# jglaser/metadynamics-plugin

Hardware: AMD Instinct MI355X
Metric: particle_cv_evals_per_s (higher is better)
Workload: dtype f32; 1 GPU; 1xMI355X: 10^6 particles, 2 lamellar CVs (8 Fourier modes each), 256^2 bias grid, well-tempered; particles_per_gpu=1000000, particles_global=1000000, n_cv=2, modes_per_cv=8, grid=256x256, stride=1, fast_trig=1, fast_trig_library_default=1, driver=host, mode=single

## Files before the change

### include/mtd_abi.h

```cpp
#ifndef MTD_ABI_H
#define MTD_ABI_H

#include <stddef.h>

#ifdef __cplusplus
extern "C" {
#endif

#define MTD_ABI_VERSION 1

typedef void *mtd_stream_t;

enum mtd_dtype { MTD_F32 = 0, MTD_F64 = 1 };

enum mtd_status
    {
    MTD_SUCCESS = 0,
    MTD_ERR_INVALID_ARGUMENT = -1,
    MTD_ERR_UNSUPPORTED = -2,
    MTD_ERR_NO_DEVICE = -3,
    MTD_ERR_COMM_TIMEOUT = -4,
    MTD_ERR_COLLECTIVE = -5
    };

// ... 70 lines not shown
                     const double *cv_max, const unsigned int *num_points, double W, double T_shift,
                     double T, unsigned int stride, int mode, int add_bias);
int mtd_metad_destroy(mtd_metad *m);

int mtd_metad_set_stride(mtd_metad *m, unsigned int stride);
int mtd_metad_set_add_hills(mtd_metad *m, int add_bias);
int mtd_metad_set_mode(mtd_metad *m, int mode);
int mtd_metad_set_sigma_inv(mtd_metad *m, const double *sigma_inv );
int mtd_metad_reset_histogram(mtd_metad *m, mtd_stream_t stream);

int mtd_metad_set_cv_source(mtd_metad *m, unsigned int cv, const double *d_partials, unsigned int n_partials,
                            unsigned int stride, unsigned int offset, double scale, double shift);

int mtd_metad_set_cv_value(mtd_metad *m, unsigned int cv, double value);

const double *mtd_metad_bias_device(const mtd_metad *m);
const double *mtd_metad_cv_device(const mtd_metad *m);

int mtd_metad_update_bias(mtd_metad *m, unsigned int timestep, mtd_stream_t stream);

int mtd_metad_update_phase_a(mtd_metad *m, unsigned int timestep, int *deposited, mtd_stream_t stream);
int mtd_metad_update_phase_b(mtd_metad *m, int deposited, mtd_stream_t stream);
int mtd_metad_delta_buffers(mtd_metad *m, double **d_real, unsigned int **d_count, unsigned int *num_elements);

int mtd_metad_get_state(mtd_metad *m, double *cv, double *bias, double *bias_potential, double *weight,
                        unsigned int *num_gaussians, unsigned int *num_out_of_bounds, mtd_stream_t stream);
double mtd_metad_sigma_determinant(const mtd_metad *m);
unsigned int mtd_metad_num_elements(const mtd_metad *m);

int mtd_metad_get_array(mtd_metad *m, int which, void *host_out, mtd_stream_t stream);
int mtd_metad_set_array(mtd_metad *m, int which, const void *host_in, mtd_stream_t stream);
int mtd_metad_set_num_gaussians(mtd_metad *m, unsigned int n, mtd_stream_t stream);
void *mtd_metad_device_array(mtd_metad *m, int which);
int mtd_metad_grid_touched(mtd_metad *m, mtd_stream_t stream);


int mtd_fused_cv_pass(mtd_metad *m, const mtd_lamellar_set *set, unsigned int n_particles, const void *d_postype,
                      int dtype, const mtd_box *global_box, double *d_partials, unsigned int *n_partials,
                      mtd_stream_t stream);

int mtd_fused_force_pass(mtd_metad *m, const mtd_lamellar_set *set, unsigned int n_particles, const void *d_postype,
                         void *const *d_force, int dtype, unsigned int n_global, const mtd_box *global_box,
                         unsigned int timestep, mtd_stream_t stream);

int mtd_fused_force_pass_slots(mtd_metad *m, const mtd_lamellar_set *set, const unsigned int *slots, unsigned int n_particles,
                               const void *d_postype, void *const *d_force, int dtype, unsigned int n_global,
                               const mtd_box *global_box, unsigned int timestep, mtd_stream_t stream);

int mtd_fused_step(mtd_metad *m, const mtd_lamellar_set *set, unsigned int n_particles, const void *d_postype,
                   void *const *d_force, int dtype, unsigned int n_global, const mtd_box *global_box, double *d_scratch,
                   unsigned int timestep, mtd_stream_t stream);
unsigned int mtd_fused_step_launches(const mtd_metad *m);
int mtd_fused_step_set_mode(mtd_metad *m, int mode);

int mtd_profile_force_begin(unsigned int n_launches);
int mtd_profile_force_end(double *durations_us, unsigned int capacity, unsigned int *n_out);

#define MTD_RCCL_ID_BYTES 128
#define MTD_ELEM_F64 1
#define MTD_ELEM_U32 2
typedef struct mtd_rccl mtd_rccl;
int mtd_rccl_unique_id(void *out_id);
int mtd_rccl_create(mtd_rccl **out, const void *unique_id, unsigned int rank, unsigned int world);
int mtd_comm_allreduce_large(mtd_rccl *r, void *d_buffer, size_t count, int elem, mtd_stream_t stream);
unsigned int mtd_rccl_world(const mtd_rccl *r);
unsigned int mtd_rccl_rank(const mtd_rccl *r);
int mtd_rccl_destroy(mtd_rccl *r);
const char *mtd_rccl_last_error(void);
int mtd_metad_update_bias_walkers(mtd_metad *m, mtd_rccl *walkers, unsigned int timestep, mtd_stream_t stream);


#define MTD_COMM_MAX_RANKS 8
#define MTD_COMM_HANDLE_BYTES 64

typedef struct mtd_comm mtd_comm;

int mtd_comm_create(mtd_comm **out, unsigned int rank, unsigned int world, unsigned int max_doubles);
int mtd_comm_handle(mtd_comm *c, void *out_handle);
int mtd_comm_connect(mtd_comm *c, const void *handles);
int mtd_comm_allreduce_small(mtd_comm *c, double *d_values, unsigned int n, mtd_stream_t stream);
int mtd_comm_status(mtd_comm *c, unsigned int *timeouts, mtd_stream_t stream);
#define MTD_COMM_MAX_SHARED 8
int mtd_comm_share(mtd_comm *c, size_t bytes, void **d_local, unsigned int *slot, void *out_handle);
int mtd_comm_open(mtd_comm *c, unsigned int slot, const void *handles, void **peers);
size_t mtd_comm_pull_bytes(size_t max_doubles);
int mtd_comm_pull_attach(mtd_comm *c, size_t max_doubles, void *const *in_peers, void *const *out_peers);
int mtd_comm_allreduce_pull(mtd_comm *c, double *d_buffer, size_t count, mtd_stream_t stream);
unsigned int mtd_comm_world(const mtd_comm *c);
unsigned int mtd_comm_rank(const mtd_comm *c);
int mtd_comm_destroy(mtd_comm *c);

int mtd_metad_set_comm(mtd_metad *m, mtd_comm *comm);


typedef struct mtd_mesh mtd_mesh;

int mtd_mesh_create(mtd_mesh **out, unsigned int nx, unsigned int ny, unsigned int nz, const double *mode,
                    unsigned int n_types, unsigned int max_particles);
int mtd_mesh_destroy(mtd_mesh *m);
int mtd_mesh_set_bug_compat(mtd_mesh *m, int on);
int mtd_mesh_set_keep_fourier(mtd_mesh *m, int on);
int mtd_mesh_set_cv_event(mtd_mesh *m, void *hip_event);
unsigned int mtd_mesh_num_cells(const mtd_mesh *m);

int mtd_mesh_compute_cv(mtd_mesh *m, unsigned int n_particles, const void *d_postype, int dtype, const mtd_box *box,
                        unsigned int n_global, const double **d_partials, unsigned int *n_partials, mtd_stream_t stream);
// ... 131 lines not shown
```

### metadynamics-plugin_amd/csrc/fused.hip

```cpp
#include <hip/hip_runtime.h>
#include <hip/hip_ext.h>

#ifdef MTD_STAMPS
__device__ unsigned long long g_stamps[64];
#define MTD_STAMP(slot, cond)                                                   \
    do                                                                          \
        {                                                                       \
        if (cond) g_stamps[slot] = wall_clock64();                              \
        } while (0)
extern "C" int mtd_debug_read_stamps(unsigned long long *host)
    {
    return (int)hipMemcpyFromSymbol(host, HIP_SYMBOL(g_stamps), sizeof(unsigned long long) * 64);
    }
#else
#define MTD_STAMP(slot, cond) do { } while (0)
#endif

#include "lamellar_host.hpp"
#include "metad_host.hpp"
#include "comm_host.hpp"

#include <cstdlib>
#include <cstring>
#include <map>
// ... 29 lines not shown
        apply_cells(c, b0, min(c.len, b0 + FCV_THREADS), blockIdx.x == 0, s_red);
        MTD_STAMP(1, blockIdx.x == 0 && threadIdx.x == 0);
        return;
        }
    const unsigned int block_id = blockIdx.x - n_apply_blocks;
    const unsigned int n_blocks = gridDim.x - n_apply_blocks;

    RawGroup<S4, U> first;
    const S4 *src = N ? postype : (const S4 *)partials;
    lam_load_group_nc<S4, U>(src, N ? N : 1u, block_id * FCV_THREADS + threadIdx.x, n_blocks * FCV_THREADS, first);
    const CvTableRegs tab = stage_cv_tables_request(a);
    stage_cv_tables_store(tab, s_coeff, s_mt);
    __syncthreads();
    MTD_STAMP(4, block_id == 0 && threadIdx.x == 0);
    float acc[NCV];
#pragma unroll
    for (int i = 0; i < NCV; ++i) acc[i] = 0.0f;
    lam_cv_accumulate<S4, NCV, FAST, U, ORTHO>(a, postype, N, block_id * FCV_THREADS + threadIdx.x, n_blocks * FCV_THREADS,
                                               s_coeff, s_mt, first, acc);
    MTD_STAMP(5, block_id == 0 && threadIdx.x == 0);
    lam_cv_block_reduce<NCV>(acc, s_wave, partials, block_id);
    MTD_STAMP(6, block_id == 0 && threadIdx.x == 0);
    if (COMM)
        {
        constexpr int NS = NCV < 3 ? NCV : 3;
        if (threadIdx.x < NS)
            ll_store(ck.ll + ((size_t)block_id * NS + threadIdx.x) * 2, ck.seq, partials[block_id * NCV + threadIdx.x]);
        if (block_id != 0 || threadIdx.x >= MTD_WAVE) return;
        double v[3] = { 0.0, 0.0, 0.0 };
        const bool expired = ll_collect_wave<NS>(ck, n_blocks, v);
        MTD_STAMP(7, threadIdx.x == 0);
        double tot[3] = { 0.0, 0.0, 0.0 };
#pragma unroll
        for (int i = 0; i < NS; ++i)
            {
            const double t = wave_sum(v[i]);
            tot[i] = expired ? comm_poison() : t;
            }
        MTD_STAMP(8, threadIdx.x == 0);
        comm_send_wave(ck, tot, NS);
        MTD_STAMP(9, threadIdx.x == 0);
        }
    }

constexpr int FF_STREAM_WAVES = FF_THREADS / MTD_WAVE - 1;
constexpr int FF_STREAM_THREADS = FF_STREAM_WAVES * MTD_WAVE;
constexpr int FF_U = 4;
template<typename S4, int NCV, bool FAST> struct ff_groups { static constexpr int value = 1; };
template<> struct ff_groups<float4, 1, true> { static constexpr int value = 2; };
template<> struct ff_groups<float4, 2, true> { static constexpr int value = 2; };
template<> struct ff_groups<float4, 1, false> { static constexpr int value = 2; };
template<> struct ff_groups<double4, 1, true> { static constexpr int value = 2; };
template<> struct ff_groups<double4, 1, false> { static constexpr int value = 2; };

template<typename S4, int NCV, bool FAST, int GROUPS, bool COMM, bool ORTHO>
__global__ __launch_bounds__(FF_THREADS, 4) void k_fused_force(const LamKArgs a, const S4 *__restrict__ postype, const ForcePtrs out,
                                                            const unsigned int N, const double two_over_n, const MetadCfg c,
                                                            const int deposit, const unsigned int n_grid_blocks, const CommK ck)
    {
    __shared__ ChainResult s_chain;
    __shared__ float s_wcoef[MTD_MAX_CV * MTD_MAX_TYPES];
    __shared__ double s_red[16];
    __shared__ ModeTables s_mt;

    const int wave = threadIdx.x >> 6;
    const int lane = threadIdx.x & 63;
    const bool grid_block = blockIdx.x < n_grid_blocks;
    const unsigned int block_id = blockIdx.x - n_grid_blocks;
    const unsigned int n_blocks = gridDim.x - n_grid_blocks;
    const unsigned int stride = n_blocks * FF_STREAM_THREADS;
    const unsigned int first = block_id * FF_STREAM_THREADS + (wave - 1) * MTD_WAVE + lane;
    const unsigned int first1 = first + FF_U * stride;

    ForceRegs<NCV, FF_U> R, R1;
    MTD_STAMP(16, blockIdx.x == 0 && threadIdx.x == 0);
    MTD_STAMP(24, blockIdx.x == n_grid_blocks && threadIdx.x == 0);
    constexpr int NCH = CHAIN_MAX_CV;
    ChainPre<NCH> pre;
    constexpr bool early = !COMM;
    float4 th = make_float4(0.f, 0.f, 0.f, 0.f), tq = th;
    float tc = 0.0f;
    if (wave == 0)
        {
        if (!grid_block)
            {
            if (lane < (int)a.n_modes)
                {
                th = a.h[lane];
                tq = a.q[lane];
                }
            if (lane < NCV * MTD_MAX_TYPES) tc = a.coeff[lane / MTD_MAX_TYPES][lane % MTD_MAX_TYPES];
            }
        if (early)
            chain_preload<NCH>(c, pre);
        else
            chain_preload<NCH, false>(c, pre);
        }
    RawGroup<S4, FF_U> raw0;
    if (wave != 0 && !grid_block && N) lam_force_request<S4, FF_U>(postype, N, first, stride, raw0);
    if (!grid_block)
        {
        if (wave == 0)
            {
            if (lane < (int)a.n_modes)
                {
                s_mt.h[lane] = th;
                s_mt.q[lane] = tq;
                }
            if (lane < NCV * MTD_MAX_TYPES) s_wcoef[lane] = tc;
            }
        lds_barrier();
        }
    MTD_STAMP(25, blockIdx.x == n_grid_blocks && threadIdx.x == 0);
    if (wave == 0)
        {
        ChainResult r;
        if constexpr (early)
            {
            double vi[3];
#pragma unroll
            for (int i = 0; i < NCH; ++i) vi[i] = (pre.x[i][0] + pre.x[i][1]) + (pre.x[i][2] + pre.x[i][3]);
            r = chain_wave(c, deposit != 0, true, nullptr, nullptr, false, &pre.patch, pre.patch_ok != 0, true, vi[0], vi[1], vi[2]);
            }
        else
            r = chain_wave(c, deposit != 0, true, &ck, nullptr, false, &pre.patch, pre.patch_ok != 0);
        MTD_STAMP(17, blockIdx.x == 0 && threadIdx.x == 0);
        MTD_STAMP(26, blockIdx.x == n_grid_blocks && threadIdx.x == 0);
        if (lane == 0) chain_share(s_chain, r);
        if (!grid_block && lane < NCV * MTD_MAX_TYPES)
            {
            const unsigned int cv = lane / MTD_MAX_TYPES;
            const unsigned int gs = cv < a.n_cv ? a.slot[cv] : 0u;
            const double b = gs == 0 ? r.bias[0] : (gs == 1 ? r.bias[1] : r.bias[2]);
            s_wcoef[lane] = (cv < a.n_cv) ? (float)((double)s_wcoef[lane] * b * two_over_n) : 0.0f;
            }
        }
    else if (!grid_block && N)
        {
        RawGroup<S4, FF_U> raw1;
        if (GROUPS > 1) lam_force_request<S4, FF_U>(postype, N, first1, stride, raw1);
        lam_force_unscaled_from<S4, NCV, FAST, FF_U, ORTHO>(a, N, first, stride, s_mt, raw0, R);
        if (GROUPS > 1) lam_force_unscaled_from<S4, NCV, FAST, FF_U, ORTHO>(a, N, first1, stride, s_mt, raw1, R1);
        MTD_STAMP(27, blockIdx.x == n_grid_blocks && threadIdx.x == 64);
        }
    lds_barrier();
    MTD_STAMP(18, blockIdx.x == 0 && threadIdx.x == 0);
    MTD_STAMP(28, blockIdx.x == n_grid_blocks && threadIdx.x == 64);

    if (grid_block)
        {
        const double2 sums = grid_first_pass_cells_256(c, s_chain, blockIdx.x);
        MTD_STAMP(19, blockIdx.x == 0 && threadIdx.x == 0);
        grid_first_pass_sums_256(c, blockIdx.x, sums, s_red);
        MTD_STAMP(20, blockIdx.x == 0 && threadIdx.x == 0);
        }
    else if (wave != 0 && N)
        {
        lam_force_store<S4, NCV, FF_U>(a, out, first, stride, s_wcoef, R);
        if (GROUPS > 1) lam_force_store<S4, NCV, FF_U>(a, out, first1, stride, s_wcoef, R1);
        MTD_STAMP(29, blockIdx.x == n_grid_blocks && threadIdx.x == 64);
        }

    if (blockIdx.x == 0 && wave == 0) publish_step(c, s_chain, deposit, nullptr, COMM ? &ck : nullptr);
    }

template<typename S4, bool FAST>
__global__ __launch_bounds__(FF_THREADS) void k_fused_force_general(const LamKArgs a, const S4 *__restrict__ postype, const ForcePtrs out,
                                                            const unsigned int N, const double two_over_n, const MetadCfg c,
                                                            const int deposit, const unsigned int n_grid_blocks)
    {
    __shared__ EvalShared sh;
    __shared__ float s_wcoef[MTD_MAX_CV * MTD_MAX_TYPES];
    __shared__ double s_red[16];
    __shared__ ModeTables s_mt;

    load_modes(a, s_mt, true);
    reduce_cv_sources(c, sh.cv, s_red);
    __syncthreads();
    evaluate_bias(c, sh, deposit != 0, true);

    if (blockIdx.x < n_grid_blocks)
        {
        const unsigned int g = blockIdx.x * FF_THREADS + threadIdx.x;
        double s1 = 0.0, s2 = 0.0;
        if (g < c.len)
            {
            const double dV = (c.W * sh.scal) * exp(-gauss_exponent(c, g, sh.cv));
            c.grid_delta[g] = dV;
            unsigned int hd = c.hist_delta[g];
            if (sh.on_grid && g == sh.bin)
                {
                hd += 1;
                c.hist_delta[g] = hd;
                c.sigma_grid_delta[g] += c.det_sigma;
                c.hist_gauss_delta[g] += 1;
                }
            const double R = c.rew[g] + (double)hd;
            c.rew[g] = R;
            s1 = R * dV;
            s2 = R;
            }
        s1 = block_sum(s1, s_red);
        s2 = block_sum(s2, s_red);
        if (threadIdx.x == 0)
            {
            c.gpart[2 * blockIdx.x] = s1;
            c.gpart[2 * blockIdx.x + 1] = s2;
            }
        }

    if (blockIdx.x == 0)
        {
        if (threadIdx.x < c.n_cv)
// ... 130 lines not shown
        MTD_LAUNCH_CHECK();
        return MTD_SUCCESS;
        });
    if (rc) return rc;
    m->pending_apply = 0;
    return MTD_SUCCESS;
    }

int mtd_fused_force_pass(mtd_metad *m, const mtd_lamellar_set *set, unsigned int n_particles, const void *d_postype,
                         void *const *d_force, int dtype, unsigned int n_global, const mtd_box *global_box,
                         unsigned int timestep, mtd_stream_t stream)
    {
    if (!m || !set) return MTD_ERR_INVALID_ARGUMENT;
    if (set->n_cv != m->cfg.n_cv) return MTD_ERR_UNSUPPORTED;
    return mtd_fused_force_pass_slots(m, set, nullptr, n_particles, d_postype, d_force, dtype, n_global, global_box, timestep, stream);
    }

int mtd_fused_force_pass_slots(mtd_metad *m, const mtd_lamellar_set *set, const unsigned int *slots, unsigned int n_particles,
                               const void *d_postype, void *const *d_force, int dtype, unsigned int n_global,
                               const mtd_box *global_box, unsigned int timestep, mtd_stream_t stream)
    {
    if (!m) return MTD_ERR_INVALID_ARGUMENT;
    LamKArgs k;
    int rc = fill_kargs(k, set, global_box);
    if (rc) return rc;
    if (!d_force || n_global == 0 || (n_particles && !d_postype)) return MTD_ERR_INVALID_ARGUMENT;
    if (dtype != MTD_F32 && dtype != MTD_F64) return MTD_ERR_INVALID_ARGUMENT;
    if (set->n_cv > m->cfg.n_cv) return MTD_ERR_UNSUPPORTED;
    if (!slots && set->n_cv != m->cfg.n_cv) return MTD_ERR_INVALID_ARGUMENT;
    if (slots)
        {
        if (m->comm) return MTD_ERR_UNSUPPORTED;
        for (unsigned int c = 0; c < set->n_cv; ++c)
            {
            if (slots[c] >= m->cfg.n_cv) return MTD_ERR_INVALID_ARGUMENT;
            k.slot[c] = (unsigned char)slots[c];
            }
        }
    hipStream_t s = (hipStream_t)stream;
    rc = metad_flush(m, s);
    if (rc) return rc;
    ForcePtrs out;
    for (unsigned int c = 0; c < MTD_MAX_CV; ++c) out.f[c] = nullptr;
    for (unsigned int c = 0; c < set->n_cv; ++c)
        {
        if (!d_force[c] && n_particles) return MTD_ERR_INVALID_ARGUMENT;
        out.f[c] = d_force[c];
        }
    const int dep = deposit_due(m, timestep);
    const unsigned int n_grid = dep ? m->cfg.n_gblocks : 0;
    const double two_over_n = 2.0 / (double)n_global;
    const bool fast = lam_fast_trig(k) != 0;
    static const bool force_general = std::getenv("MTD_FUSED_GENERAL") != nullptr;
    CommK ck;
    std::memset(&ck, 0, sizeof(ck));
    if (m->comm)
        {
        if (m->cfg.n_cv > (unsigned int)CHAIN_MAX_CV || force_general) return MTD_ERR_UNSUPPORTED;
        rc = comm_current(m->comm, ck);
        if (rc) return rc;
        }
    if (m->cfg.n_cv <= (unsigned int)CHAIN_MAX_CV && !force_general)
        {
        hipEvent_t ev_start = nullptr, ev_stop = nullptr;
        const bool timed = force_profile_next(ev_start, ev_stop);
        dispatch_s4_fast(dtype, fast, [&](auto s4, auto fast_c)
            {
            using S4 = typename decltype(s4)::type;
            constexpr bool FAST = decltype(fast_c)::value;
            dispatch_count<CHAIN_MAX_CV>(set->n_cv, [&](auto n)
                {
                constexpr int NCV = decltype(n)::value, G = ff_groups<S4, NCV, FAST>::value;
                const unsigned int per_block = FF_STREAM_THREADS * FF_U * G;
                unsigned int fblocks = (n_particles + per_block - 1) / per_block;
                if (fblocks == 0 && n_grid == 0) fblocks = 1;
                const unsigned int grid = n_grid + fblocks;
                dispatch_bool(m->comm != nullptr, [&](auto comm_c)
                    {
                    dispatch_bool(k.ortho != 0, [&](auto ortho_c)
                        {
                        const auto kernel = k_fused_force<S4, NCV, FAST, G, decltype(comm_c)::value, decltype(ortho_c)::value>;
                        if (timed)
                            hipExtLaunchKernelGGL(kernel, dim3(grid), dim3(FF_THREADS), 0, s, ev_start, ev_stop, 0, k, (const S4 *)d_postype, out,
                                                  n_particles, two_over_n, m->cfg, dep, n_grid, ck);
                        else
                            kernel<<<grid, FF_THREADS, 0, s>>>(k, (const S4 *)d_postype, out, n_particles, two_over_n, m->cfg, dep, n_grid, ck);
                        });
                    });
                });
            });
        }
    else
        {
        unsigned int fblocks = lam_force_blocks(n_particles);
        if (n_particles == 0) fblocks = n_grid ? 0 : 1;
        const unsigned int grid = n_grid + fblocks;
        dispatch_s4_fast(dtype, fast, [&](auto s4, auto fast_c)
            {
            using S4 = typename decltype(s4)::type;
            k_fused_force_general<S4, decltype(fast_c)::value><<<grid, FF_THREADS, 0, s>>>(k, (const S4 *)d_postype, out, n_particles, two_over_n,
                                                                                        m->cfg, dep, n_grid);
            });
        }
    MTD_LAUNCH_CHECK();
    m->pending_apply = dep;
    m->w_stale = dep;
    return MTD_SUCCESS;
    }

int mtd_profile_force_begin(unsigned int n_launches)
    {
    std::lock_guard<std::mutex> lock(g_force_profile_mutex);
    ForceProfile &p = g_force_profile;
    for (hipEvent_t e : p.ev) (void)hipEventDestroy(e);
    p.ev.clear();
    p.used = 0;
    for (unsigned int i = 0; i < 2 * n_launches; ++i)
        {
        hipEvent_t e = nullptr;
        MTD_HIP_TRY(hipEventCreate(&e));
        p.ev.push_back(e);
        }
    return MTD_SUCCESS;
    }

int mtd_profile_force_end(double *durations_us, unsigned int capacity, unsigned int *n_out)
    {
    ForceProfile &p = g_force_profile;
    if (!durations_us || !n_out) return MTD_ERR_INVALID_ARGUMENT;
    MTD_HIP_TRY(hipDeviceSynchronize());
    std::lock_guard<std::mutex> lock(g_force_profile_mutex);
    unsigned int n = 0;
    for (size_t i = 0; i + 1 < p.used && n < capacity; i += 2)
        {
        float ms = 0.0f;
        MTD_HIP_TRY(hipEventElapsedTime(&ms, p.ev[i], p.ev[i + 1]));
        durations_us[n++] = 1.0e3 * (double)ms;
        }
    *n_out = n;
    for (hipEvent_t e : p.ev) (void)hipEventDestroy(e);
    p.ev.clear();
    p.used = 0;
    return MTD_SUCCESS;
    }

int mtd_metad_set_comm(mtd_metad *m, mtd_comm *comm)
    {
    if (!m) return MTD_ERR_INVALID_ARGUMENT;
    if (comm && (!comm->connected || m->cfg.n_cv > (unsigned int)CHAIN_MAX_CV || comm->max_doubles < m->cfg.n_cv))
        return comm && !comm->connected ? MTD_ERR_INVALID_ARGUMENT : MTD_ERR_UNSUPPORTED;
    m->comm = comm;
    return MTD_SUCCESS;
    }

}

namespace mtd
{
int fused_grid_step(mtd_metad *m, unsigned int timestep, hipStream_t s)
    {
    if (m->cfg.n_cv > (unsigned int)CHAIN_MAX_CV) return MTD_ERR_UNSUPPORTED;
    int rc = metad_flush(m, s);
    if (rc) return rc;
    LamKArgs k;
    std::memset(&k, 0, sizeof(k));
    k.n_cv = m->cfg.n_cv;
    ForcePtrs out;
    for (unsigned int c = 0; c < MTD_MAX_CV; ++c) out.f[c] = nullptr;
    const int dep = deposit_due(m, timestep);
    const unsigned int n_grid = dep ? m->cfg.n_gblocks : 0;
    const unsigned int grid = n_grid ? n_grid : 1;
    CommK ck;
    std::memset(&ck, 0, sizeof(ck));
    switch (m->cfg.n_cv)
        {
        case 1: k_fused_force<float4, 1, true, 1, false, false><<<grid, FF_THREADS, 0, s>>>(k, nullptr, out, 0, 0.0, m->cfg, dep, n_grid, ck); break;
        case 2: k_fused_force<float4, 2, true, 1, false, false><<<grid, FF_THREADS, 0, s>>>(k, nullptr, out, 0, 0.0, m->cfg, dep, n_grid, ck); break;
        default: k_fused_force<float4, 3, true, 1, false, false><<<grid, FF_THREADS, 0, s>>>(k, nullptr, out, 0, 0.0, m->cfg, dep, n_grid, ck); break;
        }
    MTD_LAUNCH_CHECK();
    m->pending_apply = dep;
    m->w_stale = dep;
    if (dep) announce_pending_apply(m, s);
    return MTD_SUCCESS;
    }
}
```

### metadynamics-plugin_amd/csrc/lamellar_device.hpp

```cpp
#pragma once

#include "mtd_device.hpp"

namespace mtd
{

struct LamKArgs
    {
    double B[3][3];
    unsigned int n_cv, n_modes, n_types;
    unsigned int trig;
    unsigned int first[MTD_MAX_CV + 1];
    unsigned char slot[MTD_MAX_CV];
    unsigned int ortho;
    float4 h[MTD_MAX_MODES];
    unsigned char corder[MTD_MAX_MODES];
    unsigned char nact[MTD_MAX_CV];
    float4 q[MTD_MAX_MODES];
    float coeff[MTD_MAX_CV][MTD_MAX_TYPES];
    };

struct ForcePtrs
    {
    void *f[MTD_MAX_CV];
// ... 333 lines not shown
        {
#pragma unroll
        for (int pp = 0; pp < P; ++pp) R.f[pp][c][0] = R.f[pp][c][1] = R.f[pp][c][2] = (v2f)(0.0f);
        if (c < (int)a.n_cv)
            {
            const unsigned int k1 = a.first[c + 1];
#pragma unroll 4
            for (unsigned int k = a.first[c]; k < k1; ++k)
                {
                const float4 h = mt.h[k];
                const float4 q = mt.q[k];
#pragma unroll
                for (int pp = 0; pp < P; ++pp)
                    {
                    const v2f t = h.x * g0[pp] + h.y * g1[pp] + h.z * g2[pp];
                    v2f sn;
                    sn.x = sin2pi<FAST>(t.x);
                    sn.y = sin2pi<FAST>(t.y);
                    R.f[pp][c][0] += q.x * sn;
                    R.f[pp][c][1] += q.y * sn;
                    R.f[pp][c][2] += q.z * sn;
                    }
                }
            }
        }
    }

template<typename S4, int NCV, int U>
__device__ __forceinline__ void lam_force_store(const LamKArgs &a, const ForcePtrs &out, const unsigned int first,
                                                const unsigned int stride, const float *s_wcoef, const ForceRegs<NCV, U> &R)
    {
    typedef typename scalar4_traits<S4>::scalar scalar;
#pragma unroll
    for (int c = 0; c < NCV; ++c)
        {
        if (c < (int)a.n_cv)
            {
            S4 *f = (S4 *)out.f[c];
#pragma unroll
            for (int u = 0; u < U; ++u)
                {
                if (R.ok[u])
                    {
                    const float w = s_wcoef[c * MTD_MAX_TYPES + R.type[u]];
                    const S4 v = scalar4_traits<S4>::make((scalar)(R.f[u / 2][c][0][u % 2] * w), (scalar)(R.f[u / 2][c][1][u % 2] * w),
                                                          (scalar)(R.f[u / 2][c][2][u % 2] * w), (scalar)0);
                    nt_store(v, &f[first + u * stride]);
                    }
                }
            }
        }
    }

}
```

### metadynamics-plugin_amd/csrc/metad.hip

```cpp
#include "metad_device.hpp"

#include <cmath>
#include <cstring>
#include <mutex>
#include <new>

#include "metad_host.hpp"
#include "comm_host.hpp"

#include <cstdlib>

namespace
{

using namespace mtd;

__global__ __launch_bounds__(GRID_THREADS) void k_prepare(const MetadCfg c, const int deposit)
    {
    __shared__ EvalShared sh;
    __shared__ double s_tmp[16];
    reduce_cv_sources(c, sh.cv, s_tmp);
    __syncthreads();
    evaluate_bias(c, sh, deposit != 0, false);
    if (threadIdx.x < c.n_cv) c.st->cv[threadIdx.x] = sh.cv[threadIdx.x];
// ... 298 lines not shown
    unsigned long long len = 1;
    for (unsigned int i = 0; i < n_cv; ++i)
        {
        if (!(cv_min[i] < cv_max[i]) || num_points[i] < 2 || !(sigma[i] > 0.0))
            {
            delete m;
            return MTD_ERR_INVALID_ARGUMENT;
            }
        c.lengths[i] = num_points[i];
        c.factors[i] = (i == 0) ? 1 : c.lengths[i - 1] * c.factors[i - 1];
        c.cv_min[i] = cv_min[i];
        c.cv_max[i] = cv_max[i];
        c.delta[i] = (cv_max[i] - cv_min[i]) / (double)(num_points[i] - 1);
        c.sigma_inv[i * n_cv + i] = 1.0 / sigma[i];
        len *= num_points[i];
        if (len > 0x7fffffffULL)
            {
            delete m;
            return MTD_ERR_UNSUPPORTED;
            }
        }
    c.len = (unsigned int)len;
    c.W = W;
    c.T_shift = T_shift;
    c.temp = T;
    c.mode = mode;
    c.det_sigma = host_determinant(c.sigma_inv, n_cv);
    c.n_gblocks = (c.len + GRID_THREADS - 1) / GRID_THREADS;
    {
    const ExactDivisor dT = make_exact_divisor(T_shift);
    int ok = dT.fast;
    c.rT_shift = dT.y;
    for (unsigned int i = 0; i < n_cv && i < 3; ++i)
        {
        const ExactDivisor d1 = make_exact_divisor(c.delta[i]), d2 = make_exact_divisor(2.0 * c.delta[i]);
        c.rdelta[i] = d1.y;
        c.rdelta2[i] = d2.y;
        ok = ok && d1.fast && d2.fast;
        }
    c.fastdiv = ok;
    }
    m->stride = stride;
    m->add_bias = add_bias ? 1 : 0;
    m->pending_apply = 0;
    m->w_stale = 0;
    m->comm = nullptr;
    m->d_ll = nullptr;
    m->d_step_err = nullptr;
    m->h_step_err = nullptr;
    m->d_step_err_host = nullptr;
    m->step_seq = 0;
    m->last_launches = 0;
    m->step_mode = -1;
    m->walkers_checked = nullptr;
    m->walkers_stride = 0;
    m->walkers_add_bias = 0;

    const size_t G = c.len;
    const size_t bytes_d = 6 * G * sizeof(double);
    const size_t bytes_u = 4 * G * sizeof(unsigned int);
    const size_t bytes_state = (sizeof(MetadState) + 255) / 256 * 256;
    const size_t bytes_gpart = 2 * (size_t)c.n_gblocks * sizeof(double);
    const size_t total = bytes_d + bytes_u + bytes_state + bytes_gpart;
    hipError_t e = hipMalloc(&m->slab, total);
    if (e != hipSuccess)
        {
        delete m;
        return (int)e;
        }
    e = hipMemset(m->slab, 0, total);
    if (e != hipSuccess)
        {
        (void)hipFree(m->slab);
        delete m;
        return (int)e;
        }
    char *p = (char *)m->slab;
    c.grid = (double *)p;
    c.rew = c.grid + G;
    c.weight = c.rew + G;
    c.sigma_grid = c.weight + G;
    c.grid_delta = c.sigma_grid + G;
    c.sigma_grid_delta = c.grid_delta + G;
    p += bytes_d;
    c.hist = (unsigned int *)p;
    c.hist_gauss = c.hist + G;
    c.hist_delta = c.hist_gauss + G;
    c.hist_gauss_delta = c.hist_delta + G;
    p += bytes_u;
    c.st = (MetadState *)p;
    p += bytes_state;
    c.gpart = (double *)p;

    k_fill<<<(c.len + 255) / 256, 256>>>(c.weight, 1.0, c.len);
    MetadState st;
    std::memset(&st, 0, sizeof(st));
    st.w = 1.0;
    st.scal = 1.0;
    e = hipMemcpy(c.st, &st, sizeof(st), hipMemcpyHostToDevice);
    if (e == hipSuccess) e = hipDeviceSynchronize();
    if (e != hipSuccess)
        {
        (void)hipFree(m->slab);
        delete m;
        return (int)e;
        }
// ... 342 lines not shown
```

### metadynamics-plugin_amd/csrc/metad_host.hpp

```cpp
#pragma once

#include "metad_device.hpp"

struct mtd_metad
    {
    mtd::MetadCfg cfg;
    unsigned int stride;
    int add_bias;
    void *slab;
    int pending_apply;
    int w_stale;
    struct mtd_comm *comm;
    unsigned long long *d_ll;
    unsigned int *d_step_err;
    volatile unsigned int *h_step_err;
    unsigned int *d_step_err_host;
    unsigned int step_seq;
    unsigned int last_launches;
    int step_mode;
    const void *walkers_checked;
    unsigned int walkers_stride;
    int walkers_add_bias;
    };

namespace mtd
{
inline int deposit_due(const mtd_metad *m, unsigned int timestep) { return (m->add_bias && (timestep % m->stride == 0)) ? 1 : 0; }
unsigned int resident_capacity(const void *kernel, int threads);
int metad_flush(mtd_metad *m, hipStream_t s);
int fused_grid_step(mtd_metad *m, unsigned int timestep, hipStream_t s);
void announce_pending_apply(mtd_metad *m, hipStream_t s);
void withdraw_pending_apply(mtd_metad *m);
mtd_metad *take_pending_apply(hipStream_t s, MetadCfg &cfg);
void commit_pending_apply(mtd_metad *m);
void fused_step_release(mtd_metad *m);
}
```

### metadynamics-plugin_amd/metadynamics/_abi.py

```python
import ctypes as C
import os

_HERE = os.path.dirname(os.path.abspath(__file__))
PKG_ROOT = os.path.dirname(_HERE)
REPO_ROOT = os.path.dirname(PKG_ROOT)
LIB_PATH = os.environ.get("MTD_LIB_OVERRIDE") or os.path.join(PKG_ROOT, "lib", "libmtd_hip.so")
HEADER_PATH = os.path.join(REPO_ROOT, "include", "mtd_abi.h")

MTD_MAX_CV = 8
MTD_MAX_MODES = 64
MTD_MAX_TYPES = 16
MTD_METAD_MAX_CV = 6
MTD_F32, MTD_F64 = 0, 1
MODE_STANDARD, MODE_WELL_TEMPERED = 0, 1

ARRAY_NAMES = ["grid", "grid_delta", "reweighted", "weight", "sigma_grid", "sigma_grid_delta",
               "hist", "hist_delta", "hist_gauss", "hist_gauss_delta"]


class MtdError(RuntimeError):
    pass


class Box(C.Structure):
# ... 63 lines not shown
    "mtd_lamellar_scratch_doubles": (C.c_size_t, [C.c_uint]),
    "mtd_calculate_fourier_modes": (C.c_int, [C.c_uint, _ip, C.c_uint, _vp, C.c_int, _dp, C.c_uint, _vp, _vp,
                                               C.POINTER(Box), _vp]),
    "mtd_lamellar_cv_partials": (C.c_int, [C.POINTER(LamellarSet), C.c_uint, _vp, C.c_int, C.POINTER(Box), _vp,
                                            _up, _vp]),
    "mtd_reduce_partials": (C.c_int, [_vp, C.c_uint, C.c_uint, C.c_uint, C.c_double, C.c_double, _vp, _vp]),
    "mtd_compute_sq_forces": (C.c_int, [C.c_uint, _vp, _vp, C.c_int, C.c_uint, _ip, _dp, C.c_uint, C.c_uint,
                                         C.c_double, C.POINTER(Box), _vp]),
    "mtd_lamellar_forces": (C.c_int, [C.POINTER(LamellarSet), C.c_uint, _vp, C.POINTER(_vp), C.c_int, C.c_uint,
                                       _vp, C.POINTER(Box), _vp]),
    "mtd_lamellar_set_fast_trig": (C.c_int, [C.c_int]),
    "mtd_lamellar_get_fast_trig": (C.c_int, []),
    "mtd_debug_sph_harmonics": (C.c_int, [C.c_uint, C.c_uint, _vp, _vp]),
    "mtd_rccl_last_error": (C.c_char_p, []),
    "mtd_mesh_clear_rider": (C.c_int, [_vp, C.POINTER(C.c_int)]),
    "mtd_mesh_assign_info": (C.c_int, [_vp, C.POINTER(C.c_int), C.POINTER(C.c_uint), _vp]),
    "mtd_mesh_transform_info": (C.c_int, [_vp, C.POINTER(C.c_int)]),
    "mtd_mesh_forces_update_bias": (C.c_int, [_vp, _vp, C.c_uint, C.POINTER(LamellarSet), _up, C.c_uint, _vp, _vp, C.POINTER(_vp), C.c_int, C.c_uint,
                                              C.POINTER(Box), C.c_uint, _vp]),
    "mtd_mesh_set_lamellar_rider": (C.c_int, [_vp, _vp, _vp, _vp, C.c_uint, _vp, C.POINTER(C.c_uint), _vp]),
    "mtd_ql_symmetrize_half_list": (C.c_int, [C.c_uint, _vp, _vp, _vp, _vp, _vp, _vp, C.c_size_t, C.POINTER(C.c_size_t), _vp]),
    "mtd_debug_index_decode": (C.c_int, [C.c_uint, _vp, C.c_uint, _vp, _vp, _vp]),
    "mtd_update_grid": (C.c_int, [C.c_uint, _up, C.c_uint, _vp, _vp, _dp, _dp, _dp, C.c_double, C.c_double, _vp]),
    "mtd_metad_create": (C.c_int, [C.POINTER(_vp), C.c_uint, _dp, _dp, _dp, _up, C.c_double, C.c_double,
                                    C.c_double, C.c_uint, C.c_int, C.c_int]),
    "mtd_metad_destroy": (C.c_int, [_vp]),
    "mtd_metad_set_stride": (C.c_int, [_vp, C.c_uint]),
    "mtd_metad_set_add_hills": (C.c_int, [_vp, C.c_int]),
    "mtd_metad_set_mode": (C.c_int, [_vp, C.c_int]),
    "mtd_metad_set_sigma_inv": (C.c_int, [_vp, _dp]),
    "mtd_metad_reset_histogram": (C.c_int, [_vp, _vp]),
    "mtd_metad_set_cv_source": (C.c_int, [_vp, C.c_uint, _vp, C.c_uint, C.c_uint, C.c_uint, C.c_double, C.c_double]),
    "mtd_metad_set_cv_value": (C.c_int, [_vp, C.c_uint, C.c_double]),
    "mtd_metad_bias_device": (_vp, [_vp]),
    "mtd_metad_cv_device": (_vp, [_vp]),
    "mtd_metad_update_bias": (C.c_int, [_vp, C.c_uint, _vp]),
    "mtd_metad_update_phase_a": (C.c_int, [_vp, C.c_uint, _ip, _vp]),
    "mtd_metad_update_phase_b": (C.c_int, [_vp, C.c_int, _vp]),
    "mtd_metad_delta_buffers": (C.c_int, [_vp, C.POINTER(_vp), C.POINTER(_vp), _up]),
    "mtd_metad_get_state": (C.c_int, [_vp, _dp, _dp, _dp, _dp, _up, _up, _vp]),
    "mtd_metad_sigma_determinant": (C.c_double, [_vp]),
    "mtd_metad_num_elements": (C.c_uint, [_vp]),
    "mtd_metad_get_array": (C.c_int, [_vp, C.c_int, _vp, _vp]),
    "mtd_metad_set_array": (C.c_int, [_vp, C.c_int, _vp, _vp]),
    "mtd_metad_set_num_gaussians": (C.c_int, [_vp, C.c_uint, _vp]),
    "mtd_metad_device_array": (_vp, [_vp, C.c_int]),
    "mtd_fused_cv_pass": (C.c_int, [_vp, C.POINTER(LamellarSet), C.c_uint, _vp, C.c_int, C.POINTER(Box), _vp, _up, _vp]),
    "mtd_fused_force_pass": (C.c_int, [_vp, C.POINTER(LamellarSet), C.c_uint, _vp, C.POINTER(_vp), C.c_int, C.c_uint,
                                        C.POINTER(Box), C.c_uint, _vp]),
    "mtd_fused_step": (C.c_int, [_vp, C.POINTER(LamellarSet), C.c_uint, _vp, C.POINTER(_vp), C.c_int, C.c_uint, C.POINTER(Box), _vp,
                                  C.c_uint, _vp]),
    "mtd_fused_step_launches": (C.c_uint, [_vp]),
    "mtd_fused_step_set_mode": (C.c_int, [_vp, C.c_int]),
    "mtd_profile_force_begin": (C.c_int, [C.c_uint]),
    "mtd_profile_force_end": (C.c_int, [_dp, C.c_uint, _up]),
    "mtd_comm_create": (C.c_int, [C.POINTER(_vp), C.c_uint, C.c_uint, C.c_uint]),
    "mtd_comm_handle": (C.c_int, [_vp, _vp]),
    "mtd_comm_connect": (C.c_int, [_vp, _vp]),
    "mtd_comm_allreduce_small": (C.c_int, [_vp, _vp, C.c_uint, _vp]),
    "mtd_comm_status": (C.c_int, [_vp, _up, _vp]),
    "mtd_comm_share": (C.c_int, [_vp, C.c_size_t, C.POINTER(_vp), _up, _vp]),
    "mtd_comm_open": (C.c_int, [_vp, C.c_uint, _vp, C.POINTER(_vp)]),
    "mtd_comm_world": (C.c_uint, [_vp]),
    "mtd_comm_rank": (C.c_uint, [_vp]),
    "mtd_comm_destroy": (C.c_int, [_vp]),
    "mtd_metad_set_comm": (C.c_int, [_vp, _vp]),
    "mtd_rccl_unique_id": (C.c_int, [_vp]),
    "mtd_rccl_create": (C.c_int, [C.POINTER(_vp), _vp, C.c_uint, C.c_uint]),
    "mtd_comm_allreduce_large": (C.c_int, [_vp, _vp, C.c_size_t, C.c_int, _vp]),
    "mtd_rccl_world": (C.c_uint, [_vp]),
    "mtd_rccl_rank": (C.c_uint, [_vp]),
    "mtd_rccl_destroy": (C.c_int, [_vp]),
    "mtd_metad_update_bias_walkers": (C.c_int, [_vp, _vp, C.c_uint, _vp]),
    "mtd_fused_force_pass_slots": (C.c_int, [_vp, C.POINTER(LamellarSet), _up, C.c_uint, _vp, C.POINTER(_vp), C.c_int, C.c_uint,
                                              C.POINTER(Box), C.c_uint, _vp]),
    "mtd_mesh_create": (C.c_int, [C.POINTER(_vp), C.c_uint, C.c_uint, C.c_uint, _dp, C.c_uint, C.c_uint]),
    "mtd_mesh_destroy": (C.c_int, [_vp]),
    "mtd_mesh_set_bug_compat": (C.c_int, [_vp, C.c_int]),
    "mtd_mesh_set_keep_fourier": (C.c_int, [_vp, C.c_int]),
    "mtd_mesh_set_cv_event": (C.c_int, [_vp, _vp]),
    "mtd_mesh_num_cells": (C.c_uint, [_vp]),
    "mtd_mesh_set_table": (C.c_int, [_vp, _dp, _dp, C.c_uint, C.c_double, C.c_double]),
    "mtd_mesh_set_use_table": (C.c_int, [_vp, C.c_int]),
    "mtd_mesh_qmax": (C.c_int, [_vp, C.POINTER(Box), C.c_uint, _dp, _vp]),
    "mtd_mesh_virial": (C.c_int, [_vp, C.POINTER(Box), C.c_uint, C.c_double, _dp, _vp]),
    "mtd_mesh_assign": (C.c_int, [_vp, C.c_uint, _vp, C.c_int, C.POINTER(Box), _vp]),
    "mtd_mesh_exchange_buffer": (C.c_int, [_vp, C.POINTER(_vp), C.POINTER(C.c_size_t)]),
    "mtd_mesh_spectral": (C.c_int, [_vp, C.POINTER(Box), C.c_uint, C.POINTER(_vp), _up, _vp]),
    "mtd_mesh_compute_cv": (C.c_int, [_vp, C.c_uint, _vp, C.c_int, C.POINTER(Box), C.c_uint, C.POINTER(_vp), _up, _vp]),
    "mtd_mesh_forces": (C.c_int, [_vp, C.c_uint, _vp, _vp, C.c_int, C.POINTER(Box), C.c_uint, _vp, C.c_double, _vp]),
    "mtd_mesh_slab_bytes": (C.c_int, [_vp, C.c_uint, C.POINTER(C.c_size_t)]),
    "mtd_mesh_slab_attach": (C.c_int, [_vp, _vp, C.POINTER(_vp), C.POINTER(_vp), C.POINTER(_vp), C.POINTER(_vp)]),
    "mtd_mesh_slab_compute_cv": (C.c_int, [_vp, C.c_uint, _vp, C.c_int, C.POINTER(Box), C.c_uint, C.POINTER(_vp), _vp]),
    "mtd_mesh_get_array": (C.c_int, [_vp, C.c_int, _vp, _vp]),
    "mtd_ql_scratch_doubles": (C.c_size_t, [C.c_uint]),
    "mtd_ql_accumulate_local": (C.c_int, [C.c_uint, _vp, C.c_int, C.POINTER(Box), _vp, _vp, _vp, C.c_int, C.c_double, C.c_double,
                                           C.c_uint, C.c_uint, C.c_uint, _vp, C.POINTER(_vp), _up, _vp]),
    "mtd_ql_finalize": (C.c_int, [C.c_int, C.c_uint, _dp, C.c_uint, _vp, C.POINTER(_vp), C.POINTER(_vp), C.POINTER(_vp), _vp]),
    "mtd_ql_finalize_update_bias": (C.c_int, [_vp, C.c_int, C.c_uint, _dp, C.c_uint, _vp, C.c_uint, C.POINTER(_vp), C.POINTER(_vp), C.POINTER(_vp), _vp]),
    "mtd_metad_grid_touched": (C.c_int, [_vp, _vp]),
    "mtd_comm_pull_bytes": (C.c_size_t, [C.c_size_t]),
    "mtd_comm_pull_attach": (C.c_int, [_vp, C.c_size_t, C.POINTER(_vp), C.POINTER(_vp)]),
    "mtd_comm_allreduce_pull": (C.c_int, [_vp, _vp, C.c_size_t, _vp]),
    "mtd_ql_accumulate": (C.c_int, [C.c_uint, _vp, C.c_int, C.POINTER(Box), _vp, _vp, _vp, C.c_int, C.c_double, C.c_double, C.c_uint,
                                     C.c_uint, _dp, C.c_uint, _vp, C.POINTER(_vp), C.POINTER(_vp), C.POINTER(_vp), _vp]),
    "mtd_ql_set_half_list_exact": (C.c_int, [C.c_int]),
# ... 72 lines not shown
```

Before: 109.5 billion particle-CV-evals/s.

## Cap fused force grid at resident capacity and loop remaining particle groups

The fused force kernel's streaming blocks are capped by default at the number of blocks that can be resident at once, minus the grid blocks. Each block then walks any further particle groups in a persistent tail loop that prefetches the next group's positions while computing the current one. This is meant to remove multi-wave tail effects and repeated per-block setup (mode tables, chain preload) for large particle counts. The trade-off is more serial work per thread and a dependence on the occupancy query; the limit can be overridden by an API call or an environment variable.

```diff
diff --git a/include/mtd_abi.h b/include/mtd_abi.h
--- a/include/mtd_abi.h
+++ b/include/mtd_abi.h
@@ -146,6 +146,8 @@
                    unsigned int timestep, mtd_stream_t stream);
 unsigned int mtd_fused_step_launches(const mtd_metad *m);
 int mtd_fused_step_set_mode(mtd_metad *m, int mode);
+
+int mtd_fused_force_set_block_limit(mtd_metad *m, unsigned int n_blocks);
 
 int mtd_profile_force_begin(unsigned int n_launches);
 int mtd_profile_force_end(double *durations_us, unsigned int capacity, unsigned int *n_out);
diff --git a/metadynamics-plugin_amd/csrc/fused.hip b/metadynamics-plugin_amd/csrc/fused.hip
--- a/metadynamics-plugin_amd/csrc/fused.hip
+++ b/metadynamics-plugin_amd/csrc/fused.hip
@@ -105,11 +105,14 @@
 template<> struct ff_groups<float4, 1, false> { static constexpr int value = 2; };
 template<> struct ff_groups<double4, 1, true> { static constexpr int value = 2; };
 template<> struct ff_groups<double4, 1, false> { static constexpr int value = 2; };
+template<typename S4, int NCV, bool FAST> struct ff_tail_pipelined { static constexpr bool value = true; };
+template<bool FAST> struct ff_tail_pipelined<double4, 3, FAST> { static constexpr bool value = false; };
 
 template<typename S4, int NCV, bool FAST, int GROUPS, bool COMM, bool ORTHO>
 __global__ __launch_bounds__(FF_THREADS, 4) void k_fused_force(const LamKArgs a, const S4 *__restrict__ postype, const ForcePtrs out,
                                                             const unsigned int N, const double two_over_n, const MetadCfg c,
-                                                            const int deposit, const unsigned int n_grid_blocks, const CommK ck)
+                                                            const int deposit, const unsigned int n_grid_blocks, const CommK ck,
+                                                            const unsigned int n_groups)
     {
     __shared__ ChainResult s_chain;
     __shared__ float s_wcoef[MTD_MAX_CV * MTD_MAX_TYPES];
@@ -128,6 +131,7 @@
     ForceRegs<NCV, FF_U> R, R1;
     MTD_STAMP(16, blockIdx.x == 0 && threadIdx.x == 0);
     MTD_STAMP(24, blockIdx.x == n_grid_blocks && threadIdx.x == 0);
+    MTD_STAMP(30, blockIdx.x == gridDim.x - 1 && threadIdx.x == 64);
     constexpr int NCH = CHAIN_MAX_CV;
     ChainPre<NCH> pre;
     constexpr bool early = !COMM;
@@ -212,6 +216,14 @@
         lam_force_store<S4, NCV, FF_U>(a, out, first, stride, s_wcoef, R);
         if (GROUPS > 1) lam_force_store<S4, NCV, FF_U>(a, out, first1, stride, s_wcoef, R1);
         MTD_STAMP(29, blockIdx.x == n_grid_blocks && threadIdx.x == 64);
+        if (n_groups > (unsigned int)GROUPS)
+            {
+            RawGroup<S4, FF_U> tail;
+            lam_force_request_nc<S4, FF_U>(postype, N, first + GROUPS * FF_U * stride, stride, tail);
+            lam_force_tail<S4, NCV, FAST, FF_U, ORTHO, ff_tail_pipelined<S4, NCV, FAST>::value>(a, postype, out, N, first, stride, GROUPS, n_groups,
+                                                                                               s_mt, s_wcoef, tail);
+            }
+        MTD_STAMP(31, blockIdx.x == gridDim.x - 1 && threadIdx.x == 64);
         }
 
     if (blockIdx.x == 0 && wave == 0) publish_step(c, s_chain, deposit, nullptr, COMM ? &ck : nullptr);
@@ -448,6 +460,7 @@
     const double two_over_n = 2.0 / (double)n_global;
     const bool fast = lam_fast_trig(k) != 0;
     static const bool force_general = std::getenv("MTD_FUSED_GENERAL") != nullptr;
+    static const unsigned int env_limit = [] { const char *e = std::getenv("MTD_FORCE_BLOCK_LIMIT"); return e ? (unsigned int)std::strtoul(e, nullptr, 10) : 0u; }();
     CommK ck;
     std::memset(&ck, 0, sizeof(ck));
     if (m->comm)
@@ -468,19 +481,29 @@
                 {
                 constexpr int NCV = decltype(n)::value, G = ff_groups<S4, NCV, FAST>::value;
                 const unsigned int per_block = FF_STREAM_THREADS * FF_U * G;
-                unsigned int fblocks = (n_particles + per_block - 1) / per_block;
-                if (fblocks == 0 && n_grid == 0) fblocks = 1;
-                const unsigned int grid = n_grid + fblocks;
+                const unsigned int want = (n_particles + per_block - 1) / per_block;
                 dispatch_bool(m->comm != nullptr, [&](auto comm_c)
                     {
                     dispatch_bool(k.ortho != 0, [&](auto ortho_c)
                         {
                         const auto kernel = k_fused_force<S4, NCV, FAST, G, decltype(comm_c)::value, decltype(ortho_c)::value>;
+                        unsigned int limit = m->force_block_limit ? m->force_block_limit : env_limit;
+                        if (!limit)
+                            {
+                            const unsigned int cap = resident_capacity((const void *)kernel, FF_THREADS);
+                            if (cap) limit = cap > n_grid ? cap - n_grid : 1;
+                            }
+                        unsigned int fblocks = limit && want > limit ? limit : want;
+                        if (fblocks == 0 && n_grid == 0) fblocks = 1;
+                        const unsigned int grid = n_grid + fblocks;
+                        const unsigned int per_group = fblocks * FF_STREAM_THREADS * FF_U;
+                        const unsigned int n_groups = per_group ? (unsigned int)(((unsigned long long)n_particles + per_group - 1) / per_group) : 0;
                         if (timed)
                             hipExtLaunchKernelGGL(kernel, dim3(grid), dim3(FF_THREADS), 0, s, ev_start, ev_stop, 0, k, (const S4 *)d_postype, out,
-                                                  n_particles, two_over_n, m->cfg, dep, n_grid, ck);
+                                                  n_particles, two_over_n, m->cfg, dep, n_grid, ck, n_groups);
                         else
-                            kernel<<<grid, FF_THREADS, 0, s>>>(k, (const S4 *)d_postype, out, n_particles, two_over_n, m->cfg, dep, n_grid, ck);
+                            kernel<<<grid, FF_THREADS, 0, s>>>(k, (const S4 *)d_postype, out, n_particles, two_over_n, m->cfg, dep, n_grid, ck,
+                                                               n_groups);
                         });
                     });
                 });
@@ -501,6 +524,13 @@
     MTD_LAUNCH_CHECK();
     m->pending_apply = dep;
     m->w_stale = dep;
+    return MTD_SUCCESS;
+    }
+
+int mtd_fused_force_set_block_limit(mtd_metad *m, unsigned int n_blocks)
+    {
+    if (!m) return MTD_ERR_INVALID_ARGUMENT;
+    m->force_block_limit = n_blocks;
     return MTD_SUCCESS;
     }
 
@@ -570,9 +600,9 @@
     std::memset(&ck, 0, sizeof(ck));
     switch (m->cfg.n_cv)
         {
-        case 1: k_fused_force<float4, 1, true, 1, false, false><<<grid, FF_THREADS, 0, s>>>(k, nullptr, out, 0, 0.0, m->cfg, dep, n_grid, ck); break;
-        case 2: k_fused_force<float4, 2, true, 1, false, false><<<grid, FF_THREADS, 0, s>>>(k, nullptr, out, 0, 0.0, m->cfg, dep, n_grid, ck); break;
-        default: k_fused_force<float4, 3, true, 1, false, false><<<grid, FF_THREADS, 0, s>>>(k, nullptr, out, 0, 0.0, m->cfg, dep, n_grid, ck); break;
+        case 1: k_fused_force<float4, 1, true, 1, false, false><<<grid, FF_THREADS, 0, s>>>(k, nullptr, out, 0, 0.0, m->cfg, dep, n_grid, ck, 0); break;
+        case 2: k_fused_force<float4, 2, true, 1, false, false><<<grid, FF_THREADS, 0, s>>>(k, nullptr, out, 0, 0.0, m->cfg, dep, n_grid, ck, 0); break;
+        default: k_fused_force<float4, 3, true, 1, false, false><<<grid, FF_THREADS, 0, s>>>(k, nullptr, out, 0, 0.0, m->cfg, dep, n_grid, ck, 0); break;
         }
     MTD_LAUNCH_CHECK();
     m->pending_apply = dep;
diff --git a/metadynamics-plugin_amd/csrc/lamellar_device.hpp b/metadynamics-plugin_amd/csrc/lamellar_device.hpp
--- a/metadynamics-plugin_amd/csrc/lamellar_device.hpp
+++ b/metadynamics-plugin_amd/csrc/lamellar_device.hpp
@@ -409,4 +409,43 @@
         }
     }
 
+template<typename S4, int U>
+__device__ __forceinline__ void lam_force_request_nc(const S4 *__restrict__ postype, const unsigned int N, const unsigned int first,
+                                                     const unsigned int stride, RawGroup<S4, U> &raw)
+    {
+#pragma unroll
+    for (int u = 0; u < U; ++u)
+        {
+        const unsigned int i = first + u * stride;
+        raw.v[u] = postype[i < N ? i : N - 1];
+        }
+    }
+
+template<typename S4, int NCV, bool FAST, int U, bool ORTHO, bool PIPE>
+__device__ __forceinline__ void lam_force_tail(const LamKArgs &a, const S4 *__restrict__ postype, const ForcePtrs &out,
+                                               const unsigned int N, const unsigned int first, const unsigned int stride,
+                                               const unsigned int g0, const unsigned int n_groups, const ModeTables &mt,
+                                               const float *s_wcoef, RawGroup<S4, U> cur)
+    {
+    unsigned int base = first + g0 * U * stride;
+    for (unsigned int g = g0; g < n_groups; ++g, base += U * stride)
+        {
+        ForceRegs<NCV, U> R;
+        if (PIPE)
+            {
+            RawGroup<S4, U> nxt;
+            lam_force_request_nc<S4, U>(postype, N, base + U * stride, stride, nxt);
+            lam_force_unscaled_from<S4, NCV, FAST, U, ORTHO>(a, N, base, stride, mt, cur, R);
+            lam_force_store<S4, NCV, U>(a, out, base, stride, s_wcoef, R);
+            cur = nxt;
+            }
+        else
+            {
+            if (g != g0) lam_force_request_nc<S4, U>(postype, N, base, stride, cur);
+            lam_force_unscaled_from<S4, NCV, FAST, U, ORTHO>(a, N, base, stride, mt, cur, R);
+            lam_force_store<S4, NCV, U>(a, out, base, stride, s_wcoef, R);
+            }
+        }
+    }
+
 }
diff --git a/metadynamics-plugin_amd/csrc/metad.hip b/metadynamics-plugin_amd/csrc/metad.hip
--- a/metadynamics-plugin_amd/csrc/metad.hip
+++ b/metadynamics-plugin_amd/csrc/metad.hip
@@ -374,6 +374,7 @@
     m->step_seq = 0;
     m->last_launches = 0;
     m->step_mode = -1;
+    m->force_block_limit = 0;
     m->walkers_checked = nullptr;
     m->walkers_stride = 0;
     m->walkers_add_bias = 0;
diff --git a/metadynamics-plugin_amd/csrc/metad_host.hpp b/metadynamics-plugin_amd/csrc/metad_host.hpp
--- a/metadynamics-plugin_amd/csrc/metad_host.hpp
+++ b/metadynamics-plugin_amd/csrc/metad_host.hpp
@@ -17,6 +17,7 @@
     unsigned int *d_step_err_host;
     unsigned int step_seq;
     unsigned int last_launches;
+    unsigned int force_block_limit;
     int step_mode;
     const void *walkers_checked;
     unsigned int walkers_stride;
diff --git a/metadynamics-plugin_amd/metadynamics/_abi.py b/metadynamics-plugin_amd/metadynamics/_abi.py
--- a/metadynamics-plugin_amd/metadynamics/_abi.py
+++ b/metadynamics-plugin_amd/metadynamics/_abi.py
@@ -139,6 +139,7 @@
                                   C.c_uint, _vp]),
     "mtd_fused_step_launches": (C.c_uint, [_vp]),
     "mtd_fused_step_set_mode": (C.c_int, [_vp, C.c_int]),
+    "mtd_fused_force_set_block_limit": (C.c_int, [_vp, C.c_uint]),
     "mtd_profile_force_begin": (C.c_int, [C.c_uint]),
     "mtd_profile_force_end": (C.c_int, [_dp, C.c_uint, _up]),
     "mtd_comm_create": (C.c_int, [C.POINTER(_vp), C.c_uint, C.c_uint, C.c_uint]),
```

New measurement: 108.8 billion particle-CV-evals/s. About the same (-0.6%).
